# YukinoriMatsuoka/indy-plenum

Hardware: AMD Instinct MI355X
Metric: Ed25519 verifies/sec at 1/8 MI355X (256B msgs) + % of INT32 VALU peak vs host CPU (higher is better)
Workload: dtype int32

## Files before the change

include/edv_measure.h:

```cpp
#ifndef EDV_MEASURE_H
#define EDV_MEASURE_H

#include <stdint.h>

#ifdef __cplusplus
extern "C" {
#endif

int edv_time_batch_dev(const uint8_t *d_sigs, const uint8_t *d_pks, const uint8_t *d_msgs,
                       const uint64_t *d_msg_off, uint64_t msg_base, uint64_t n, uint8_t *d_accept, int device,
                       int iters, float *ms_out);

int edv_profile_batch_dev(const uint8_t *d_sigs, const uint8_t *d_pks, const uint8_t *d_msgs,
                          const uint64_t *d_msg_off, uint64_t msg_base, uint64_t n, uint8_t *d_accept, int device,
                          int iters, float *ms_prep, float *ms_main);

int edv_profile_batch_dev_flush(const uint8_t *d_sigs, const uint8_t *d_pks, const uint8_t *d_msgs,
                                const uint64_t *d_msg_off, uint64_t msg_base, uint64_t n, uint8_t *d_accept,
                                int device, int iters, uint64_t flush_bytes, float *ms_prep, float *ms_flush,
                                float *ms_main);

int edv_profile_prep_sides(const uint8_t *d_sigs, const uint8_t *d_pks, const uint8_t *d_msgs,
                           const uint64_t *d_msg_off, uint64_t msg_base, uint64_t n, uint8_t *d_accept, int device,
                           int iters, float ms[5]);

int edv_test_fail_async(int device, int64_t ticket);

#define EDV_PROBE_FE_MUL 1
#define EDV_PROBE_FE_SQ 2
#define EDV_PROBE_FE_SQ2 3
#define EDV_PROBE_FE_SQ_FLOOR 4
#define EDV_PROBE_FE_TOBYTES 5
#define EDV_PROBE_FE_FROMBYTES 6
#define EDV_PROBE_FE_INVERT_SAFEGCD 7
#define EDV_PROBE_FE_POW22523 8
#define EDV_PROBE_SC_REDUCE 9
#define EDV_PROBE_HALF_SCALARS 10
#define EDV_PROBE_RECODE5 11
#define EDV_PROBE_APPROX_DIV 12
#define EDV_PROBE_FDIV_FLOOR 13
#define EDV_PROBE_EUCLID_DIV 14
#define EDV_PROBE_GE_FROMBYTES 15
#define EDV_PROBE_QUAD_SQ_SHIFT 16
#define EDV_PROBE_QUAD_DBL 17
#define EDV_PROBE_QUAD_ADD 18
#define EDV_PROBE_QUAD_CACHED 19
#define EDV_PROBE_QUAD_CACHED_SIGNED 20
#define EDV_PROBE_SC_MULADD 21
#define EDV_PROBE_RECODE8 22
#define EDV_PROBE_SCALARMULT_BASE 23
#define EDV_PROBE_GE_P3_TOBYTES 24
int edv_probe_math(int device, int op, const void *in, uint64_t in_stride, void *out, uint64_t out_stride, uint64_t n);

#define EDV_STAGE_CAP 4096
#define EDV_STAGE_SENTINEL 0xA5
#define EDV_STAGE_BUCKETS 1u
#define EDV_STAGE_SPLIT 2u
#define EDV_STAGE_PRIO 4u
#define EDV_TABLE_SET_COMPACT 0
#define EDV_TABLE_SET_LARGE 1
#define EDV_TABLE_SET_COMB 2
int edv_probe_prep_state(int device, const uint8_t *sigs, const uint8_t *pks, const uint8_t *msgs,
                         const uint64_t *msg_off, uint64_t n, int set, int side0, int nsides, uint32_t flags,
                         uint32_t *dig, uint8_t *alive, int32_t *atab, int32_t *rtab, uint32_t *perm,
                         uint8_t *accept, uint64_t *cap);
int edv_probe_main_state(int device, uint64_t n, uint64_t cap, const uint32_t *dig, const uint8_t *alive,
                         const int32_t *atab, const int32_t *rtab, const uint32_t *perm, uint32_t flags,
                         uint8_t *accept);
int edv_probe_table(int device, int set, const int32_t *tj, uint64_t n, int32_t *out);

#define EDV_LAT_RTL 0
#define EDV_LAT_QUAD 1
int edv_probe_latency_phase1(int device, int kernel, int set, const uint8_t *sigs, const uint8_t *pks,
                             const uint8_t *msgs, const uint64_t *msg_off, uint64_t n, uint32_t *dig, int32_t *pt,
                             uint8_t *ok, uint8_t *accept);
int edv_probe_latency_walk(int device, int kernel, uint64_t n, uint64_t slots, const uint32_t *dig, const int32_t *pt,
                           const uint8_t *ok, uint32_t flags, uint8_t *accept);

#ifdef __cplusplus
}
#endif
#endif
```

indy-plenum_amd/csrc/edv_hostcheck.cpp:

```cpp
#define EDV_CHAIN_FLOOR 1
#include <stdint.h>
#include <string.h>
#include <vector>
#include "edv_verify_core.h"
#include "edv_sha256.h"
#include "edv_merkle.h"
#include "edv_ledger.h"
#include "edv_tables.h"
#include "edv_hostplan.h"
#include "edv_selftest_cases.h"
#include "edv_probe_ops.h"

using namespace edv;

namespace {
struct HostATab {
  ge_cached t[kAEntries];
  int staged = 0;
  void store(int e, const ge_cached& c) { t[e] = c; }
  ge_cached load(int e) const { return t[e]; }
  void stage(int e) { staged = e; }
  ge_cached fetch() const { return t[staged]; }
};
struct HostBTab {
// ... 139 lines not shown
  bool neg = false;
  half_scalars(h, a, u, neg);
  store_words(a32, a, 8);
  store_words(u32, u, 8);
  return neg ? 1 : 0;
}
int hc_probe_math(int op, const void* in, uint64_t in_stride, void* out, uint64_t out_stride, uint64_t n) {
  const ProbeSize sz = probe_size(op);
  if (!sz.in || probe_is_quad(op) || in_stride < sz.in || out_stride < sz.out || (in_stride & 3) || (out_stride & 3))
    return -1;
  for (uint64_t i = 0; i < n; i++) {
    const uint32_t* x = reinterpret_cast<const uint32_t*>(static_cast<const uint8_t*>(in) + i * in_stride);
    uint32_t* y = reinterpret_cast<uint32_t*>(static_cast<uint8_t*>(out) + i * out_stride);
    switch (op) {
#define HC_PROBE_CASE(OP) case OP: probe_lane_op<OP>(x, y); break;
      HC_PROBE_CASE(EDV_PROBE_FE_MUL)
      HC_PROBE_CASE(EDV_PROBE_FE_SQ)
      HC_PROBE_CASE(EDV_PROBE_FE_SQ2)
      HC_PROBE_CASE(EDV_PROBE_FE_SQ_FLOOR)
      HC_PROBE_CASE(EDV_PROBE_FE_TOBYTES)
      HC_PROBE_CASE(EDV_PROBE_FE_FROMBYTES)
      HC_PROBE_CASE(EDV_PROBE_FE_INVERT_SAFEGCD)
      HC_PROBE_CASE(EDV_PROBE_FE_POW22523)
      HC_PROBE_CASE(EDV_PROBE_SC_REDUCE)
      HC_PROBE_CASE(EDV_PROBE_HALF_SCALARS)
      HC_PROBE_CASE(EDV_PROBE_RECODE5)
      HC_PROBE_CASE(EDV_PROBE_APPROX_DIV)
      HC_PROBE_CASE(EDV_PROBE_FDIV_FLOOR)
      HC_PROBE_CASE(EDV_PROBE_EUCLID_DIV)
      HC_PROBE_CASE(EDV_PROBE_GE_FROMBYTES)
      HC_PROBE_CASE(EDV_PROBE_SC_MULADD)
      HC_PROBE_CASE(EDV_PROBE_RECODE8)
      HC_PROBE_CASE(EDV_PROBE_GE_P3_TOBYTES)
#undef HC_PROBE_CASE
      case EDV_PROBE_SCALARMULT_BASE: probe_scalarmult_base(x, y, comb()); break;
      default: return -1;
    }
  }
  return 0;
}
static_assert(kAEntries * 40 == 360, "a slot's table is 9 entries of 4 x 10 limbs");
int hc_stage_prep(const uint8_t* sigs, const uint8_t* pks, const uint8_t* msgs, const uint64_t* off, uint64_t n,
                  int bits, int side0, int nsides, int buckets, uint64_t cap, uint32_t* dig, uint8_t* alive,
                  int32_t* atab, int32_t* rtab, uint32_t* perm, uint8_t* accept) {
  if ((bits != kBBits && bits != kBBitsCompact) || n > cap || side0 < 0 || nsides < 1 || side0 + nsides > 3) return -1;
  const HostBTab& bt = btab(bits);
  if (buckets) {
    auto bucket = [&](uint64_t i) {
      const uint64_t nb = (64 + (off[i + 1] - off[i]) + 17 + 127) / 128;
      return nb < 63 ? nb : uint64_t(63);
    };
    uint64_t k = 0;
    bool one = true;
    for (uint64_t i = 1; i < n; i++) one = one && bucket(i) == bucket(0);
    for (uint64_t b = 0; b < 64 && !one; b++)
      for (uint64_t i = 0; i < n; i++)
        if (bucket(i) == b) perm[k++] = uint32_t(i);
    for (uint64_t i = 0; one && i < n; i++) perm[i] = uint32_t(i);
  }
  for (uint64_t j = 0; j < n; j++) {
    const uint64_t i = buckets ? perm[j] : j;
    uint32_t R[8], S[8], A[8];
    load_words(R, sigs + 64 * i, 8);
    load_words(S, sigs + 64 * i + 32, 8);
    load_words(A, pks + 32 * i, 8);
    for (int side = side0; side < side0 + nsides; side++) {
// ... 492 lines not shown
```

indy-plenum_amd/csrc/edv_math.h:

```cpp
#pragma once
#include <stdint.h>

#if defined(__HIPCC__)
#include <hip/hip_runtime.h>
#define EDV_HD __host__ __device__ __forceinline__
#else
#define EDV_HD inline
#endif

namespace edv {

struct fe { int32_t v[10]; };

EDV_HD fe fe_d() { return fe{{56195235, 13857412, 51736253, 6949390, 114729, 24766616, 60832955, 30306712, 48412415, 21499315}}; }
EDV_HD fe fe_d2() { return fe{{45281625, 27714825, 36363642, 13898781, 229458, 15978800, 54557047, 27058993, 29715967, 9444199}}; }
EDV_HD fe fe_sqrtm1() { return fe{{34513072, 25610706, 9377949, 3500415, 12389472, 33281959, 41962654, 31548777, 326685, 11406482}}; }

EDV_HD fe fe_zero() { return fe{{0, 0, 0, 0, 0, 0, 0, 0, 0, 0}}; }
EDV_HD fe fe_one() { return fe{{1, 0, 0, 0, 0, 0, 0, 0, 0, 0}}; }

EDV_HD fe fe_add(const fe& f, const fe& g) {
  fe h;
#pragma unroll
  for (int i = 0; i < 10; i++) h.v[i] = f.v[i] + g.v[i];
// ... 17 lines not shown
  for (int i = 0; i < 10; i++) h.v[i] = take_b ? b.v[i] : a.v[i];
  return h;
}

template <int W>
EDV_HD int32_t carry_step(int64_t h, int64_t& next) {
  const int64_t t = h + (int64_t(1) << (W - 1));
  next += t >> W;
  return int32_t(uint32_t(t) & ((1u << W) - 1)) - (1 << (W - 1));
}

EDV_HD fe fe_carry64(int64_t h0, int64_t h1, int64_t h2, int64_t h3, int64_t h4, int64_t h5, int64_t h6,
                     int64_t h7, int64_t h8, int64_t h9) {
  h0 = carry_step<26>(h0, h1);
  h4 = carry_step<26>(h4, h5);
  h1 = carry_step<25>(h1, h2);
  h5 = carry_step<25>(h5, h6);
  h2 = carry_step<26>(h2, h3);
  h6 = carry_step<26>(h6, h7);
  h3 = carry_step<25>(h3, h4);
  h7 = carry_step<25>(h7, h8);
  h4 = carry_step<26>(h4, h5);
  h8 = carry_step<26>(h8, h9);
  int64_t c9 = 0;
  h9 = carry_step<25>(h9, c9);
  h0 += c9 * 19;
  h0 = carry_step<26>(h0, h1);
  return fe{{int32_t(h0), int32_t(h1), int32_t(h2), int32_t(h3), int32_t(h4), int32_t(h5), int32_t(h6),
             int32_t(h7), int32_t(h8), int32_t(h9)}};
}

EDV_HD constexpr int64_t col_bias(int k) { return (k & 1) ? (int64_t(1) << 24) : (int64_t(1) << 25); }
#if defined(__HIP_DEVICE_COMPILE__)
__constant__ int64_t c_col_bias[3] = {int64_t(1) << 25, int64_t(1) << 24, 0};
EDV_HD int64_t bias_reg(int k) { return c_col_bias[k & 1]; }
EDV_HD int64_t zero_reg() { return c_col_bias[2]; }
#else
EDV_HD int64_t bias_reg(int k) { return col_bias(k); }
EDV_HD int64_t zero_reg() { return 0; }
#endif
template <int W>
EDV_HD int32_t carry_biased(int64_t t, int64_t& next) {
  next += t >> W;
  return int32_t(uint32_t(t) & ((1u << W) - 1)) - (1 << (W - 1));
}
EDV_HD fe fe_carry64_biased(int64_t h0, int64_t h1, int64_t h2, int64_t h3, int64_t h4, int64_t h5, int64_t h6,
                            int64_t h7, int64_t h8, int64_t h9) {
  h0 = carry_biased<26>(h0, h1);
  h1 = carry_biased<25>(h1, h2);
  h2 = carry_biased<26>(h2, h3);
  h3 = carry_biased<25>(h3, h4);
  h4 = carry_biased<26>(h4, h5);
  h5 = carry_biased<25>(h5, h6);
  h6 = carry_biased<26>(h6, h7);
  h7 = carry_biased<25>(h7, h8);
  h8 = carry_biased<26>(h8, h9);
  int64_t c9 = 0;
  h9 = carry_biased<25>(h9, c9);
  h0 += c9 * 19;
  h0 = carry_step<26>(h0, h1);
  return fe{{int32_t(h0), int32_t(h1), int32_t(h2), int32_t(h3), int32_t(h4), int32_t(h5), int32_t(h6),
             int32_t(h7), int32_t(h8), int32_t(h9)}};
}

EDV_HD void sched_fence() {
#if defined(__HIP_DEVICE_COMPILE__) && !defined(EDV_NO_SCHED_FENCE)
  __builtin_amdgcn_sched_barrier(0);
#endif
}

struct fe_mul_cols {
  int32_t f[10], g[10], g19[10], f2[10], f38_9;
  EDV_HD fe_mul_cols(const fe& ff, const fe& gg) {
#pragma unroll
    for (int i = 0; i < 10; i++) {
      f[i] = ff.v[i];
      g[i] = gg.v[i];
      g19[i] = 19 * gg.v[i];
      f2[i] = (i & 1) ? 2 * ff.v[i] : ff.v[i];
    }
    f38_9 = 38 * ff.v[9];
  }
  EDV_HD int64_t col(int k, int64_t start) const {
    int64_t acc = 0;
#pragma unroll
    for (int i = 0; i < 10; i++) {
      const int j = k - i;
      const bool f9w = (i == 9) && (j < 0) && ((j + 10) & 1);
      const int32_t a = f9w ? f38_9 : ((k & 1) == 0) ? f2[i] : f[i];
      const int32_t b = f9w ? g[j + 10] : (j >= 0) ? g[j] : g19[j + 10];
      acc = int64_t(a) * int64_t(b) + ((i == 0) ? start : acc);
    }
    return acc;
  }
};
EDV_HD fe fe_mul(const fe& f, const fe& g) {
  sched_fence();
  const fe_mul_cols cols(f, g);
  int64_t h[10];
#pragma unroll
  for (int k = 0; k < 10; k++) h[k] = cols.col(k, bias_reg(k));
  const fe r = fe_carry64_biased(h[0], h[1], h[2], h[3], h[4], h[5], h[6], h[7], h[8], h[9]);
  sched_fence();
  return r;
}

struct sq_split { int8_t x, y; };
constexpr sq_split kSqSplit[2][10][10] = {
    {
        {{1, 1}, {1, 2}, {1, 2}, {2, 1}, {2, 1}, {2, 1}, {2, 1}, {2, 1}, {2, 1}, {2, 1}},
        {{0, 0}, {1, 2}, {2, 1}, {2, 2}, {2, 1}, {2, 2}, {1, 2}, {2, 2}, {2, 1}, {2, 38}},
        {{0, 0}, {0, 0}, {1, 1}, {1, 2}, {2, 1}, {1, 2}, {1, 2}, {1, 2}, {2, 19}, {1, 38}},
        {{0, 0}, {0, 0}, {0, 0}, {1, 2}, {2, 1}, {2, 2}, {2, 1}, {2, 38}, {2, 19}, {2, 38}},
        {{0, 0}, {0, 0}, {0, 0}, {0, 0}, {1, 1}, {1, 2}, {2, 19}, {1, 38}, {2, 19}, {1, 38}},
        {{0, 0}, {0, 0}, {0, 0}, {0, 0}, {0, 0}, {19, 2}, {2, 19}, {2, 38}, {2, 19}, {2, 38}},
        {{0, 0}, {0, 0}, {0, 0}, {0, 0}, {0, 0}, {0, 0}, {19, 1}, {1, 38}, {2, 19}, {1, 38}},
        {{0, 0}, {0, 0}, {0, 0}, {0, 0}, {0, 0}, {0, 0}, {0, 0}, {1, 38}, {2, 19}, {2, 38}},
        {{0, 0}, {0, 0}, {0, 0}, {0, 0}, {0, 0}, {0, 0}, {0, 0}, {0, 0}, {1, 19}, {1, 38}},
        {{0, 0}, {0, 0}, {0, 0}, {0, 0}, {0, 0}, {0, 0}, {0, 0}, {0, 0}, {0, 0}, {1, 38}},
    },
    {
        {{1, 2}, {1, 4}, {2, 2}, {1, 4}, {2, 2}, {2, 2}, {2, 2}, {2, 2}, {2, 2}, {1, 4}},
        {{0, 0}, {4, 1}, {4, 1}, {8, 1}, {4, 1}, {8, 1}, {1, 4}, {4, 2}, {4, 1}, {8, 19}},
        {{0, 0}, {0, 0}, {2, 1}, {1, 4}, {2, 2}, {4, 1}, {2, 2}, {4, 1}, {4, 19}, {4, 19}},
        {{0, 0}, {0, 0}, {0, 0}, {1, 4}, {1, 4}, {4, 2}, {1, 4}, {4, 38}, {4, 19}, {4, 38}},
// ... 78 lines not shown
    c = t >> w;
  }
  c9 = c;
#else
  int64_t h[10];
  fe_sq_cols<false, false>(f, h);
  o[0] = carry_floor<26>(h[0], h[1]);
  o[1] = carry_floor<25>(h[1], h[2]);
  o[2] = carry_floor<26>(h[2], h[3]);
  o[3] = carry_floor<25>(h[3], h[4]);
  o[4] = carry_floor<26>(h[4], h[5]);
  o[5] = carry_floor<25>(h[5], h[6]);
  o[6] = carry_floor<26>(h[6], h[7]);
  o[7] = carry_floor<25>(h[7], h[8]);
  o[8] = carry_floor<26>(h[8], h[9]);
  o[9] = carry_floor<25>(h[9], c9);
#endif
  int64_t t0 = int64_t(o[0]) + 19 * c9, t1 = o[1];
  o[0] = carry_floor<26>(t0, t1);
  o[1] = int32_t(t1);
  const fe r{{o[0], o[1], o[2], o[3], o[4], o[5], o[6], o[7], o[8], o[9]}};
  sched_fence();
  return r;
}
EDV_HD fe fe_sq2(const fe& f) {
  sched_fence();
  int64_t h[10];
  fe_sq_cols<true>(f, h);
  const fe r = fe_carry64_biased(h[0], h[1], h[2], h[3], h[4], h[5], h[6], h[7], h[8], h[9]);
  sched_fence();
  return r;
}

EDV_HD fe fe_carry32(const fe& f) {
  int64_t h[10];
#pragma unroll
  for (int i = 0; i < 10; i++) h[i] = f.v[i];
  return fe_carry64(h[0], h[1], h[2], h[3], h[4], h[5], h[6], h[7], h[8], h[9]);
}

EDV_HD void fe_tobytes(uint32_t w[8], const fe& f) {
  int32_t h[10];
#pragma unroll
  for (int i = 0; i < 10; i++) h[i] = f.v[i];
  int32_t q = (19 * h[9] + (1 << 24)) >> 25;
#pragma unroll
  for (int i = 0; i < 10; i++) q = (h[i] + q) >> ((i & 1) ? 25 : 26);
  h[0] += 19 * q;
#pragma unroll
  for (int i = 0; i < 9; i++) {
    const int s = (i & 1) ? 25 : 26;
    const int32_t c = h[i] >> s;
    h[i + 1] += c;
    h[i] -= c * (1 << s);
  }
  h[9] &= (1 << 25) - 1;
  const uint32_t u0 = h[0], u1 = h[1], u2 = h[2], u3 = h[3], u4 = h[4], u5 = h[5], u6 = h[6], u7 = h[7],
                 u8 = h[8], u9 = h[9];
  w[0] = u0 | (u1 << 26);
  w[1] = (u1 >> 6) | (u2 << 19);
  w[2] = (u2 >> 13) | (u3 << 13);
  w[3] = (u3 >> 19) | (u4 << 6);
  w[4] = u5 | (u6 << 25);
  w[5] = (u6 >> 7) | (u7 << 19);
  w[6] = (u7 >> 13) | (u8 << 12);
  w[7] = (u8 >> 20) | (u9 << 6);
// ... 158 lines not shown
#pragma unroll 1
  for (int it = 0; it < 20; it++) {
    int32_t t[4];
    eta = divsteps_30(eta, uint32_t(f.v[0]), uint32_t(g.v[0]), t);
    update_de(d, e, t);
    update_fg(f, g, t);
  }
  const int64_t sgn = (f.v[8] >> 31) | 1;
  constexpr int kPos[10] = {0, 26, 51, 77, 102, 128, 153, 179, 204, 230};
  int64_t h[10] = {0, 0, 0, 0, 0, 0, 0, 0, 0, 0};
#pragma unroll
  for (int i = 0; i < 9; i++) {
    const int pos = 30 * i;
    int k = 0;
#pragma unroll
    for (int j = 0; j < 10; j++)
      if (kPos[j] <= pos) k = j;
    h[k] += (sgn * int64_t(d.v[i])) * (int64_t(1) << (pos - kPos[k]));
  }
  return fe_carry64(h[0], h[1], h[2], h[3], h[4], h[5], h[6], h[7], h[8], h[9]);
}

struct ge_p2 { fe X, Y, Z; };
struct ge_p3 { fe X, Y, Z, T; };
struct ge_p1p1 { fe X, Y, Z, T; };
struct ge_cached { fe YpX, YmX, Z, T2d; };
struct ge_precomp { fe ypx, ymx, xy2d; };

EDV_HD ge_p2 ge_p2_identity() { return ge_p2{fe_zero(), fe_one(), fe_one()}; }
EDV_HD ge_p3 ge_p3_identity() { return ge_p3{fe_zero(), fe_one(), fe_one(), fe_zero()}; }
EDV_HD ge_cached ge_cached_identity() { return ge_cached{fe_one(), fe_one(), fe_one(), fe_zero()}; }
EDV_HD ge_precomp ge_precomp_identity() { return ge_precomp{fe_one(), fe_one(), fe_zero()}; }

EDV_HD ge_p2 ge_p1p1_to_p2(const ge_p1p1& p) {
  return ge_p2{fe_mul(p.X, p.T), fe_mul(p.Z, p.Y), fe_mul(p.Z, p.T)};
}
EDV_HD ge_p3 ge_p1p1_to_p3(const ge_p1p1& p) {
  return ge_p3{fe_mul(p.X, p.T), fe_mul(p.Z, p.Y), fe_mul(p.Z, p.T), fe_mul(p.X, p.Y)};
}
EDV_HD ge_p2 ge_p3_to_p2(const ge_p3& p) { return ge_p2{p.X, p.Y, p.Z}; }
EDV_HD ge_cached ge_p3_to_cached(const ge_p3& p) {
  return ge_cached{fe_add(p.Y, p.X), fe_sub(p.Y, p.X), p.Z, fe_mul(p.T, fe_d2())};
}

EDV_HD ge_p1p1 ge_p2_dbl(const ge_p2& p) {
  ge_p1p1 r;
  const fe XX = fe_sq(p.X);
  const fe YY = fe_sq(p.Y);
  const fe B = fe_sq2(p.Z);
  const fe A = fe_sq(fe_add(p.X, p.Y));
  r.Y = fe_add(YY, XX);
  r.Z = fe_sub(YY, XX);
  r.X = fe_sub(A, r.Y);
  r.T = fe_sub(B, r.Z);
  return r;
}
EDV_HD ge_p1p1 ge_add(const ge_p3& p, const ge_cached& q) {
  ge_p1p1 r;
  const fe A = fe_mul(fe_add(p.Y, p.X), q.YpX);
  const fe B = fe_mul(fe_sub(p.Y, p.X), q.YmX);
  const fe C = fe_mul(q.T2d, p.T);
  const fe ZZ = fe_mul(p.Z, q.Z);
  const fe D = fe_add(ZZ, ZZ);
  r.X = fe_sub(A, B);
  r.Y = fe_add(A, B);
  r.Z = fe_add(D, C);
  r.T = fe_sub(D, C);
  return r;
}
EDV_HD ge_p1p1 ge_madd(const ge_p3& p, const ge_precomp& q) {
  ge_p1p1 r;
  const fe A = fe_mul(fe_add(p.Y, p.X), q.ypx);
  const fe B = fe_mul(fe_sub(p.Y, p.X), q.ymx);
  const fe C = fe_mul(q.xy2d, p.T);
  const fe D = fe_add(p.Z, p.Z);
  r.X = fe_sub(A, B);
  r.Y = fe_add(A, B);
  r.Z = fe_add(D, C);
  r.T = fe_sub(D, C);
  return r;
}
EDV_HD void fe_cswap_mask(fe& a, fe& b, int32_t m) {
#pragma unroll
  for (int i = 0; i < 10; i++) {
    const int32_t t = (a.v[i] ^ b.v[i]) & m;
    a.v[i] ^= t;
    b.v[i] ^= t;
  }
}
EDV_HD fe fe_cneg_mask(const fe& a, int32_t m) {
  fe h;
#pragma unroll
  for (int i = 0; i < 10; i++) h.v[i] = (a.v[i] ^ m) - m;
  return h;
}
// ... 267 lines not shown
```

indy-plenum_amd/csrc/edv_probe.hip:

```cpp
#define EDV_CHAIN_FLOOR 1
#include <hip/hip_runtime.h>
#include <stdint.h>

#include "edv_probe.h"

namespace edv {
namespace {

template <int OP>
__global__ __launch_bounds__(256) void edv_probe_lane_kernel(const uint8_t* in, uint64_t in_stride, uint8_t* out,
                                                             uint64_t out_stride, uint64_t n) {
  const uint64_t i = uint64_t(blockIdx.x) * 256 + threadIdx.x;
  if (i >= n) return;
  probe_lane_op<OP>(reinterpret_cast<const uint32_t*>(in + i * in_stride),
                    reinterpret_cast<uint32_t*>(out + i * out_stride));
}

__global__ __launch_bounds__(256) void edv_probe_comb_kernel(const uint8_t* in, uint64_t in_stride, uint8_t* out,
                                                             uint64_t out_stride, uint64_t n, const int32_t* comb) {
  const uint64_t i = uint64_t(blockIdx.x) * 256 + threadIdx.x;
  if (i >= n) return;
  probe_scalarmult_base(reinterpret_cast<const uint32_t*>(in + i * in_stride),
                        reinterpret_cast<uint32_t*>(out + i * out_stride), GlobalComb{comb});
}

}

hipError_t launch_probe_lane(hipStream_t s, int op, const uint8_t* in, uint64_t in_stride, uint8_t* out,
                             uint64_t out_stride, uint64_t n, const int32_t* comb) {
  const dim3 grid(unsigned((n + 255) / 256)), block(256);
  switch (op) {
    case EDV_PROBE_SCALARMULT_BASE:
      if (!comb) return hipErrorInvalidValue;
      edv_probe_comb_kernel<<<grid, block, 0, s>>>(in, in_stride, out, out_stride, n, comb);
      break;
#define EDV_PROBE_CASE(OP) \
  case OP: edv_probe_lane_kernel<OP><<<grid, block, 0, s>>>(in, in_stride, out, out_stride, n); break;
    EDV_PROBE_CASE(EDV_PROBE_FE_MUL)
    EDV_PROBE_CASE(EDV_PROBE_FE_SQ)
    EDV_PROBE_CASE(EDV_PROBE_FE_SQ2)
    EDV_PROBE_CASE(EDV_PROBE_FE_SQ_FLOOR)
    EDV_PROBE_CASE(EDV_PROBE_FE_TOBYTES)
    EDV_PROBE_CASE(EDV_PROBE_FE_FROMBYTES)
    EDV_PROBE_CASE(EDV_PROBE_FE_INVERT_SAFEGCD)
    EDV_PROBE_CASE(EDV_PROBE_FE_POW22523)
    EDV_PROBE_CASE(EDV_PROBE_SC_REDUCE)
    EDV_PROBE_CASE(EDV_PROBE_HALF_SCALARS)
    EDV_PROBE_CASE(EDV_PROBE_RECODE5)
    EDV_PROBE_CASE(EDV_PROBE_APPROX_DIV)
    EDV_PROBE_CASE(EDV_PROBE_FDIV_FLOOR)
    EDV_PROBE_CASE(EDV_PROBE_EUCLID_DIV)
    EDV_PROBE_CASE(EDV_PROBE_GE_FROMBYTES)
    EDV_PROBE_CASE(EDV_PROBE_SC_MULADD)
    EDV_PROBE_CASE(EDV_PROBE_RECODE8)
    EDV_PROBE_CASE(EDV_PROBE_GE_P3_TOBYTES)
#undef EDV_PROBE_CASE
    default: return hipErrorInvalidValue;
  }
  return hipGetLastError();
}

}
```

indy-plenum_amd/csrc/edv_probe_ops.h:

```cpp
#pragma once
#include "edv_verify_core.h"
#include "../../include/edv_measure.h"

namespace edv {

struct ProbeSize {
  uint32_t in, out;
};
EDV_HD constexpr ProbeSize probe_size(int op) {
  switch (op) {
    case EDV_PROBE_FE_MUL: return ProbeSize{80, 40};
    case EDV_PROBE_FE_SQ:
    case EDV_PROBE_FE_SQ2:
    case EDV_PROBE_FE_SQ_FLOOR:
    case EDV_PROBE_FE_INVERT_SAFEGCD:
    case EDV_PROBE_FE_POW22523: return ProbeSize{40, 40};
    case EDV_PROBE_FE_TOBYTES: return ProbeSize{40, 32};
    case EDV_PROBE_FE_FROMBYTES: return ProbeSize{32, 40};
    case EDV_PROBE_SC_REDUCE: return ProbeSize{64, 32};
    case EDV_PROBE_HALF_SCALARS: return ProbeSize{32, 68};
    case EDV_PROBE_RECODE5: return ProbeSize{32, 36};
    case EDV_PROBE_APPROX_DIV:
    case EDV_PROBE_FDIV_FLOOR: return ProbeSize{16, 8};
    case EDV_PROBE_EUCLID_DIV: return ProbeSize{128, 64};
    case EDV_PROBE_GE_FROMBYTES: return ProbeSize{32, 172};
    case EDV_PROBE_QUAD_SQ_SHIFT: return ProbeSize{176, 160};
    case EDV_PROBE_QUAD_DBL:
    case EDV_PROBE_QUAD_CACHED: return ProbeSize{160, 160};
    case EDV_PROBE_QUAD_ADD: return ProbeSize{320, 160};
    case EDV_PROBE_QUAD_CACHED_SIGNED: return ProbeSize{164, 160};
    case EDV_PROBE_SC_MULADD: return ProbeSize{96, 32};
    case EDV_PROBE_RECODE8: return ProbeSize{32, 32};
    case EDV_PROBE_SCALARMULT_BASE: return ProbeSize{32, 192};
    case EDV_PROBE_GE_P3_TOBYTES: return ProbeSize{160, 32};
    default: return ProbeSize{0, 0};
  }
}
EDV_HD constexpr bool probe_is_quad(int op) { return op >= EDV_PROBE_QUAD_SQ_SHIFT && op <= EDV_PROBE_QUAD_CACHED_SIGNED; }

EDV_HD fe probe_fe(const uint32_t* x) {
  fe f;
#pragma unroll
  for (int i = 0; i < 10; i++) f.v[i] = int32_t(x[i]);
  return f;
}
EDV_HD void probe_put(uint32_t* y, const fe& f) {
#pragma unroll
  for (int i = 0; i < 10; i++) y[i] = uint32_t(f.v[i]);
}
EDV_HD ge_p3 probe_p3(const uint32_t* x) { return ge_p3{probe_fe(x), probe_fe(x + 10), probe_fe(x + 20), probe_fe(x + 30)}; }
EDV_HD void probe_put_p3(uint32_t* y, const ge_p3& p) {
  probe_put(y, p.X);
  probe_put(y + 10, p.Y);
  probe_put(y + 20, p.Z);
  probe_put(y + 30, p.T);
}
EDV_HD double probe_f64(const uint32_t* x) { return __builtin_bit_cast(double, pack64(x[0], x[1])); }
EDV_HD void probe_put_f64(uint32_t* y, double d) {
  const uint64_t b = __builtin_bit_cast(uint64_t, d);
  y[0] = uint32_t(b);
  y[1] = uint32_t(b >> 32);
}

template <int OP>
EDV_HD void probe_lane_op(const uint32_t* x, uint32_t* y) {
  if constexpr (OP == EDV_PROBE_FE_MUL) {
    probe_put(y, fe_mul(probe_fe(x), probe_fe(x + 10)));
  } else if constexpr (OP == EDV_PROBE_FE_SQ) {
    probe_put(y, fe_sq(probe_fe(x)));
  } else if constexpr (OP == EDV_PROBE_FE_SQ2) {
    probe_put(y, fe_sq2(probe_fe(x)));
  } else if constexpr (OP == EDV_PROBE_FE_SQ_FLOOR) {
    probe_put(y, fe_sq_floor(probe_fe(x)));
  } else if constexpr (OP == EDV_PROBE_FE_TOBYTES) {
    uint32_t w[8];
    fe_tobytes(w, probe_fe(x));
#pragma unroll
    for (int i = 0; i < 8; i++) y[i] = w[i];
  } else if constexpr (OP == EDV_PROBE_FE_FROMBYTES) {
    uint32_t w[8];
#pragma unroll
    for (int i = 0; i < 8; i++) w[i] = x[i];
    probe_put(y, fe_frombytes(w));
  } else if constexpr (OP == EDV_PROBE_FE_INVERT_SAFEGCD) {
    probe_put(y, fe_invert_safegcd(probe_fe(x)));
  } else if constexpr (OP == EDV_PROBE_FE_POW22523) {
    probe_put(y, fe_pow22523(probe_fe(x)));
  } else if constexpr (OP == EDV_PROBE_SC_REDUCE) {
    uint32_t w[16], o[8];
#pragma unroll
    for (int i = 0; i < 16; i++) w[i] = x[i];
    sc_reduce(o, w);
#pragma unroll
    for (int i = 0; i < 8; i++) y[i] = o[i];
  } else if constexpr (OP == EDV_PROBE_HALF_SCALARS) {
    uint32_t h[8], a[8], u[8];
#pragma unroll
    for (int i = 0; i < 8; i++) h[i] = x[i];
    bool neg = false;
    half_scalars(h, a, u, neg);
#pragma unroll
    for (int i = 0; i < 8; i++) { y[i] = a[i]; y[8 + i] = u[i]; }
    y[16] = neg ? 1u : 0u;
  } else if constexpr (OP == EDV_PROBE_RECODE5) {
    uint32_t s[8], d[8];
#pragma unroll
// ... 62 lines not shown
```

indy-plenum_amd/csrc/edv_verify.hip:

```cpp
#include <hip/hip_runtime.h>
#include <stdint.h>

#include "edv_verify_core.h"
#include "edv_kernels.h"
#include "edv_launch.h"
#include "edv_sha256.h"

using namespace edv;

namespace {

constexpr int kEntryPieces = 10;
constexpr int kLdsAWords = kEntryPieces * 256;
constexpr int kLdsWaveWords = 2 * kLdsAWords;
__device__ __forceinline__ void wait_staged() { asm volatile("s_waitcnt vmcnt(0)" ::: "memory"); }
struct LdsATab {
  const int32_t* slot;
  int32_t* lds;
  int lane;
  __device__ __forceinline__ void stage(int e) {
    const int32_t* g = slot + e * kEntryWords;
#pragma unroll
    for (int q = 0; q < kEntryPieces; q++)
      __builtin_amdgcn_global_load_lds(const_cast<int32_t*>(g + 4 * q), lds + q * 256, 16, 0, 0);
  }
  __device__ __forceinline__ ge_cached fetch() {
    wait_staged();
    int32_t t[4 * kEntryPieces];
#pragma unroll
    for (int q = 0; q < kEntryPieces; q++) {
      const int4 v = reinterpret_cast<const int4*>(lds + q * 256)[lane];
      t[4 * q] = v.x; t[4 * q + 1] = v.y; t[4 * q + 2] = v.z; t[4 * q + 3] = v.w;
// ... 2 lines not shown
#pragma unroll
    for (int l = 0; l < 10; l++) {
      c.YpX.v[l] = t[l]; c.YmX.v[l] = t[10 + l]; c.Z.v[l] = t[20 + l]; c.T2d.v[l] = t[30 + l];
    }
    return c;
  }
};
#define EDV_MAIN_BODY \
  const uint64_t j = uint64_t(blockIdx.x) * kBlock + threadIdx.x; \
  const bool live = j < a.n && a.st.alive[j] && a.st.alive[a.st.cap + j] && a.st.alive[2 * a.st.cap + j]; \
  const uint32_t* d = a.st.dig + j; \
  const uint64_t cap = a.st.cap; \
  const uint32_t wf = live ? d[uint64_t(kDigNwin) * cap] : 0; \
  int nwin = int(wf & 0xff); \
_Pragma("unroll") \
  for (int o = 32; o > 0; o >>= 1) nwin = max(nwin, __shfl_xor(nwin, o)); \
  nwin = __builtin_amdgcn_readfirstlane(nwin); \
  if (!live) return; \
  const uint64_t i = a.base + (a.st.perm ? a.st.perm[j] : j); \
  uint32_t da[8], db[8]; \
_Pragma("unroll") \
  for (int k = 0; k < 8; k++) { \
    da[k] = d[uint64_t(k) * cap]; \
    db[k] = d[uint64_t(8 + k) * cap]; \
  } \
_Pragma("unroll") \
  for (int k = 0; k < 8; k++) { \
    da[k] = uint32_t(opaque_i32(int32_t(da[k]))); \
    db[k] = uint32_t(opaque_i32(int32_t(db[k]))); \
  } \
  int32_t* wl = lds_main + (threadIdx.x >> 6) * kLdsWaveWords; \
  const int lane = int(threadIdx.x & 63); \
  LdsATab at{a.st.atab + j * kAWords, wl, lane}, rt{a.st.rtab + j * kAWords, wl + kLdsAWords, lane}; \
  a.accept[i] = main_one(da, db, nwin, (wf >> 8) & 1, at, rt) ? 1 : 0;

__global__ __launch_bounds__(kBlock) void edv_main_kernel(VerifyArgs a) {
  __shared__ int32_t lds_main[(kBlock / 64) * kLdsWaveWords];
  EDV_MAIN_BODY
}

constexpr int kSplitMainPrio = 2;
__global__ __launch_bounds__(kBlock) void edv_main_kernel_prio(VerifyArgs a) {
  __shared__ int32_t lds_main[(kBlock / 64) * kLdsWaveWords];
  __builtin_amdgcn_s_setprio(kSplitMainPrio);
  EDV_MAIN_BODY
}

__global__ __launch_bounds__(kBlock) void edv_sign_kernel(const uint32_t* seeds, const uint8_t* msgs,
                                                          const uint64_t* off, uint64_t msg_base, uint64_t n,
                                                          uint32_t* pks, uint32_t* sigs, const int32_t* comb) {
  const uint64_t i = uint64_t(blockIdx.x) * kBlock + threadIdx.x;
  if (i >= n) return;
  uint32_t seed[8], pk[8], sig[16];
  load_words(seed, seeds + 8 * i, 2);
  const uint64_t o0 = off[i] - msg_base, o1 = off[i + 1] - msg_base;
  sign_one(pk, sig, seed, msgs + o0, o1 - o0, GlobalComb{comb});
  uint4* po = reinterpret_cast<uint4*>(pks + 8 * i);
  uint4* so = reinterpret_cast<uint4*>(sigs + 16 * i);
  po[0] = make_uint4(pk[0], pk[1], pk[2], pk[3]);
  po[1] = make_uint4(pk[4], pk[5], pk[6], pk[7]);
#pragma unroll
  for (int k = 0; k < 4; k++) so[k] = make_uint4(sig[4 * k], sig[4 * k + 1], sig[4 * k + 2], sig[4 * k + 3]);
}

__global__ void edv_comb_kernel(int32_t* out) {
  const int t = threadIdx.x + blockIdx.x * blockDim.x;
  if (t < kCombRows * kCombEntries) comb_entry(out + t * kBStride, t / kCombEntries, t % kCombEntries);
// ... 127 lines not shown
```

indy-plenum_amd/csrc/edv_verify_core.h:

```cpp
#pragma once
#include "edv_math.h"

namespace edv {

constexpr int kAWin = 4;
constexpr int kAWindows = (255 + kAWin - 1) / kAWin;
constexpr int kAEntries = (1 << (kAWin - 1)) + 1;
constexpr int kBBits = 22;
constexpr int kBTables = (253 + kBBits - 1) / kBBits;
constexpr int kBEntries = (1 << (kBBits - 1)) + 1;
constexpr int kBBitsCompact = 16;
constexpr int kBTablesCompact = (253 + kBBitsCompact - 1) / kBBitsCompact;
constexpr int kBEntriesCompact = (1 << (kBBitsCompact - 1)) + 1;
static_assert(253 - kBBits * (kBTables - 1) <= kBBits - 1, "top [S]B digit out of table range");
static_assert(253 - kBBitsCompact * (kBTablesCompact - 1) <= kBBitsCompact - 1, "top [S]B digit out of table range");
struct SbShape {
  int bits, tables, entries;
};
EDV_HD constexpr SbShape sb_large() { return SbShape{kBBits, kBTables, kBEntries}; }
EDV_HD constexpr SbShape sb_compact() { return SbShape{kBBitsCompact, kBTablesCompact, kBEntriesCompact}; }
constexpr int kCombEntries = 129;
constexpr int kBStride = 32;

EDV_HD int mx(int a, int b) { return a > b ? a : b; }
// ... 523 lines not shown
  auto next_digit = [&](bool top) {
    int e = int(s[0] & ((1u << bits) - 1)) + carry;
    shr256_var(s, bits);
    carry = top ? 0 : (e + (1 << (bits - 1))) >> bits;
    return e - carry * (1 << bits);
  };
  int dt = next_digit(sh.tables == 1);
  bt.stage(0, dt < 0 ? -dt : dt);
#pragma unroll 1
  for (int t = 0; t < sh.tables; t++) {
    const ge_precomp e = ge_precomp_cneg(bt.fetch(), dt < 0);
    if (t + 1 < sh.tables) {
      dt = next_digit(t + 2 == sh.tables);
      bt.stage(t + 1, dt < 0 ? -dt : dt);
    }
    q = ge_p1p1_to_p3(ge_madd(q, e));
  }
}
template <class BTab>
EDV_HD bool rpoint_q(const uint32_t R[8], const uint32_t S[8], BTab& bt, ge_p3& q) {
  if (!ge_is_canonical(R) || has_small_order(R)) return false;
  if (!ge_frombytes_negate(q, R)) return false;
  add_sb(q, S, bt);
  return true;
}
template <class ATab, class BTab>
EDV_HD bool prep_rpoint(const uint32_t R[8], const uint32_t S[8], ATab& tab, BTab& bt) {
  ge_p3 q;
  if (!rpoint_q(R, S, bt, q)) return false;
  build_table_projective(tab, q, bt);
  return true;
}

template <class ATab>
EDV_HD bool main_one(uint32_t da[8], uint32_t db[8], int nwin, bool negR, ATab& at, ATab& rt) {
  constexpr int kTop = kAWin * (kAWindows - 1);
  constexpr int kTopShl = 32 - kAWin - (kTop - 224);
#pragma unroll 1
  for (int k = nwin; k < kAWindows; k++) {
    shl256<kAWin>(da);
    shl256<kAWin>(db);
  }
  ge_p2 acc = ge_p2_identity();
#pragma unroll 1
  for (int w = nwin - 1; w >= 0; --w) {
    const int dA = int32_t(da[7] << kTopShl) >> (32 - kAWin);
    const int dR = int32_t(db[7] << kTopShl) >> (32 - kAWin);
    shl256<kAWin>(da);
    shl256<kAWin>(db);
    at.stage(dA < 0 ? -dA : dA);
    rt.stage(dR < 0 ? -dR : dR);
    ge_p3 p3;
    if (w == nwin - 1) {
      p3 = ge_p3_identity();
    } else {
#pragma unroll 1
      for (int d = 0; d < kAWin - 1; d++) acc = ge_p1p1_to_p2(ge_p2_dbl(acc));
      p3 = ge_p1p1_to_p3(ge_p2_dbl(acc));
    }
    const ge_cached ea = at.fetch();
    p3 = ge_p1p1_to_p3(ge_add(p3, ge_cached_cneg(ea, dA < 0)));
    const ge_cached er = rt.fetch();
    acc = ge_p1p1_to_p2(ge_add(p3, ge_cached_cneg(er, (dR < 0) != negR)));
  }
  return fe_iszero(acc.X) && fe_iszero(fe_carry32(fe_sub(acc.Y, acc.Z)));
}

template <class ATab, class BTab>
EDV_HD bool verify_one(const uint32_t R[8], const uint32_t S[8], const uint32_t A[8], const uint8_t* m, uint64_t mlen,
                       ATab& at, ATab& rt, BTab& bt) {
  PrepDigits pd;
  if (!prep_one(R, S, A, m, mlen, pd)) return false;
  if (!prep_point(A, at) || !prep_rpoint(R, S, rt, bt)) return false;
  return main_one(pd.da, pd.db, pd.nwin, pd.negR, at, rt);
}

constexpr int kCombRows = 32;
EDV_HD void comb_entry(int32_t* o, int i, int j) {
  const uint32_t Bw[8] = {0x66666658u, 0x66666666u, 0x66666666u, 0x66666666u,
                          0x66666666u, 0x66666666u, 0x66666666u, 0x66666666u};
  ge_p3 nB;
  ge_frombytes_negate(nB, Bw);
  ge_p3 base{fe_neg(nB.X), nB.Y, nB.Z, fe_neg(nB.T)};
  for (int k = 0; k < 8 * i; k++) base = ge_p1p1_to_p3(ge_p2_dbl(ge_p3_to_p2(base)));
  const ge_cached bc = ge_p3_to_cached(base);
  ge_p3 acc = ge_p3_identity();
  for (int bit = 7; bit >= 0; bit--) {
    acc = ge_p1p1_to_p3(ge_p2_dbl(ge_p3_to_p2(acc)));
    if ((j >> bit) & 1) acc = ge_p1p1_to_p3(ge_add(acc, bc));
  }
  const fe zi = fe_invert(acc.Z);
  const fe x = fe_mul(acc.X, zi), y = fe_mul(acc.Y, zi);
  const fe ypx = fe_carry32(fe_add(y, x)), ymx = fe_carry32(fe_sub(y, x));
  const fe xy2d = fe_mul(fe_mul(x, y), fe_d2());
  for (int l = 0; l < 10; l++) { o[l] = ypx.v[l]; o[10 + l] = ymx.v[l]; o[20 + l] = xy2d.v[l]; }
  o[30] = 0;
// ... 65 lines not shown
```

indy-plenum_amd/edv.py:

```python
import ctypes
import os
import threading

import numpy as np

from . import _edvhost

_HERE = os.path.dirname(os.path.abspath(__file__))
LIB_PATH = os.environ.get("EDV_LIB", os.path.join(_HERE, "libedv.so"))
MEASURE_LIB_PATH = os.path.join(_HERE, "libedv_measure.so")
MEASUREMENT_TAG = "MEASUREMENT-ONLY"

EDV_OK = 0
EDV_E_ARG = -1
EDV_E_NODEV = -2
EDV_E_HIP = -3
EDV_E_OOM = -4
EDV_E_BUSY = -5
EDV_E_SELFTEST = -6
TABLES_AUTO, TABLES_COMPACT, TABLES_LARGE = 0, 1, 2
SELFTEST_RTL, SELFTEST_TWO_WALK, SELFTEST_BATCH = 1, 2, 4
SELFTEST_ALL = 7
PREPARE_ASYNC = 1
FLAG_UNIFORM_LENGTH = 1
# ... 730 lines not shown
def profile_device(d_sigs, d_pks, d_msgs, d_off, n, d_accept, device=0, iters=1, msg_base=0):
    a, b = ctypes.c_float(0), ctypes.c_float(0)
    _mcheck(measure_lib().edv_profile_batch_dev(d_sigs, d_pks, d_msgs, d_off, msg_base, n, d_accept, device, iters,
                                                ctypes.byref(a), ctypes.byref(b)))
    return float(a.value), float(b.value)


def profile_device_flush(d_sigs, d_pks, d_msgs, d_off, n, d_accept, device=0, iters=1, flush_bytes=0, msg_base=0):
    a, f, b = ctypes.c_float(0), ctypes.c_float(0), ctypes.c_float(0)
    _mcheck(measure_lib().edv_profile_batch_dev_flush(d_sigs, d_pks, d_msgs, d_off, msg_base, n, d_accept, device,
                                                      iters, flush_bytes, ctypes.byref(a), ctypes.byref(f),
                                                      ctypes.byref(b)))
    return float(a.value), float(f.value), float(b.value)


PREP_SIDE_KEYS = ("hash_side", "a_side", "r_side", "all_three", "point_sides")


def profile_prep_sides(d_sigs, d_pks, d_msgs, d_off, n, d_accept, device=0, iters=1, msg_base=0) -> dict:
    ms = (ctypes.c_float * 5)()
    _mcheck(measure_lib().edv_profile_prep_sides(d_sigs, d_pks, d_msgs, d_off, msg_base, n, d_accept, device, iters,
                                                 ms))
    return dict(zip(PREP_SIDE_KEYS, (float(x) for x in ms)))


PROBE_OPS = {
    "fe_mul": (1, 80, 40), "fe_sq": (2, 40, 40), "fe_sq2": (3, 40, 40), "fe_sq_floor": (4, 40, 40),
    "fe_tobytes": (5, 40, 32), "fe_frombytes": (6, 32, 40), "fe_invert_safegcd": (7, 40, 40),
    "fe_pow22523": (8, 40, 40), "sc_reduce": (9, 64, 32), "half_scalars": (10, 32, 68), "recode5": (11, 32, 36),
    "approx_div": (12, 16, 8), "fdiv_floor": (13, 16, 8), "euclid_div": (14, 128, 64),
    "ge_frombytes": (15, 32, 172), "quad_sq_shift": (16, 176, 160), "quad_dbl": (17, 160, 160),
    "quad_add": (18, 320, 160), "quad_cached": (19, 160, 160), "quad_cached_signed": (20, 164, 160),
    "sc_muladd": (21, 96, 32), "recode8": (22, 32, 32), "scalarmult_base": (23, 32, 192),
    "ge_p3_tobytes": (24, 160, 32),
}


def probe_math(op, cases, device=0):
    code, nin, nout = PROBE_OPS[op]
    cases = np.ascontiguousarray(cases, dtype=np.uint8)
    if cases.ndim != 2 or cases.shape[1] != nin:
        raise ValueError("probe {}: cases must be (n, {}) bytes".format(op, nin))
    out = np.zeros((cases.shape[0], nout), np.uint8)
    _mcheck(measure_lib().edv_probe_math(device, code, cases.ctypes.data, nin, out.ctypes.data, nout,
                                         cases.shape[0]))
    return out


STAGE_CAP = 4096
STAGE_SENTINEL = 0xA5
STAGE_BUCKETS, STAGE_SPLIT, STAGE_PRIO = 1, 2, 4
TABLE_SETS = {"compact": 0, "large": 1, "comb": 2}
A_WORDS = 360
DIG_WORDS = 17


def probe_prep_state(sigs, pks, msgs, offsets, table_set="compact", buckets=False, split=False, side0=0, nsides=3,
                     device=0) -> dict:
    sigs, pks, msgs = (np.ascontiguousarray(np.frombuffer(bytes(x), np.uint8) if isinstance(x, (bytes, bytearray))
                                            else x, dtype=np.uint8) for x in (sigs, pks, msgs))
    off = np.ascontiguousarray(offsets, dtype=np.uint64)
    n = len(off) - 1
    if sigs.size != 64 * n or pks.size != 32 * n or (n and msgs.size < int(off[-1])):
        raise ValueError("prep probe: sigs n x 64, pks n x 32, msgs at least offsets[n] bytes")
    cap = ctypes.c_uint64(0)
    st = {"dig": np.full((DIG_WORDS, STAGE_CAP), STAGE_SENTINEL * 0x01010101, np.uint32),
          "alive": np.full((3, STAGE_CAP), STAGE_SENTINEL, np.uint8),
# ... 88 lines not shown
```

Measured before the change: 99.41 million.

## Interleave pairs of field multiplies and squarings in the double-scalar walk

Adds paired field multiply and square routines that accumulate two independent products column by column with a shared biased carry chain. They replace the separate fe_mul/fe_sq calls in point doubling, addition and coordinate conversions in the main verify walk, enabled by default via EDV_PAIR_PRODUCTS. The aim is more instruction-level parallelism and fewer carry passes per product, at the cost of more live registers, which can lower occupancy or cause spills.

```diff
diff --git a/include/edv_measure.h b/include/edv_measure.h
--- a/include/edv_measure.h
+++ b/include/edv_measure.h
@@ -50,6 +50,9 @@
 #define EDV_PROBE_RECODE8 22
 #define EDV_PROBE_SCALARMULT_BASE 23
 #define EDV_PROBE_GE_P3_TOBYTES 24
+#define EDV_PROBE_FE_MUL_PAIR 32
+#define EDV_PROBE_FE_SQ_PAIR 33
+#define EDV_PROBE_FE_SQ2_SQ_PAIR 34
 int edv_probe_math(int device, int op, const void *in, uint64_t in_stride, void *out, uint64_t out_stride, uint64_t n);
 
 #define EDV_STAGE_CAP 4096
diff --git a/indy-plenum_amd/csrc/edv_hostcheck.cpp b/indy-plenum_amd/csrc/edv_hostcheck.cpp
--- a/indy-plenum_amd/csrc/edv_hostcheck.cpp
+++ b/indy-plenum_amd/csrc/edv_hostcheck.cpp
@@ -195,6 +195,9 @@
       HC_PROBE_CASE(EDV_PROBE_SC_MULADD)
       HC_PROBE_CASE(EDV_PROBE_RECODE8)
       HC_PROBE_CASE(EDV_PROBE_GE_P3_TOBYTES)
+      HC_PROBE_CASE(EDV_PROBE_FE_MUL_PAIR)
+      HC_PROBE_CASE(EDV_PROBE_FE_SQ_PAIR)
+      HC_PROBE_CASE(EDV_PROBE_FE_SQ2_SQ_PAIR)
 #undef HC_PROBE_CASE
       case EDV_PROBE_SCALARMULT_BASE: probe_scalarmult_base(x, y, comb()); break;
       default: return -1;
diff --git a/indy-plenum_amd/csrc/edv_math.h b/indy-plenum_amd/csrc/edv_math.h
--- a/indy-plenum_amd/csrc/edv_math.h
+++ b/indy-plenum_amd/csrc/edv_math.h
@@ -73,12 +73,14 @@
 
 EDV_HD constexpr int64_t col_bias(int k) { return (k & 1) ? (int64_t(1) << 24) : (int64_t(1) << 25); }
 #if defined(__HIP_DEVICE_COMPILE__)
-__constant__ int64_t c_col_bias[3] = {int64_t(1) << 25, int64_t(1) << 24, 0};
+__constant__ int64_t c_col_bias[4] = {int64_t(1) << 25, int64_t(1) << 24, 0, (int64_t(1) << 25) + (int64_t(1) << 50)};
 EDV_HD int64_t bias_reg(int k) { return c_col_bias[k & 1]; }
 EDV_HD int64_t zero_reg() { return c_col_bias[2]; }
+EDV_HD int64_t pair_bias_reg() { return c_col_bias[3]; }
 #else
 EDV_HD int64_t bias_reg(int k) { return col_bias(k); }
 EDV_HD int64_t zero_reg() { return 0; }
+EDV_HD int64_t pair_bias_reg() { return col_bias(0) + (col_bias(1) << 26); }
 #endif
 template <int W>
 EDV_HD int32_t carry_biased(int64_t t, int64_t& next) {
@@ -122,16 +124,18 @@
     }
     f38_9 = 38 * ff.v[9];
   }
+  static constexpr int count(int) { return 10; }
+  EDV_HD int64_t term(int k, int i) const {
+    const int j = k - i;
+    const bool f9w = (i == 9) && (j < 0) && ((j + 10) & 1);
+    const int32_t a = f9w ? f38_9 : ((k & 1) == 0) ? f2[i] : f[i];
+    const int32_t b = f9w ? g[j + 10] : (j >= 0) ? g[j] : g19[j + 10];
+    return int64_t(a) * int64_t(b);
+  }
   EDV_HD int64_t col(int k, int64_t start) const {
     int64_t acc = 0;
 #pragma unroll
-    for (int i = 0; i < 10; i++) {
-      const int j = k - i;
-      const bool f9w = (i == 9) && (j < 0) && ((j + 10) & 1);
-      const int32_t a = f9w ? f38_9 : ((k & 1) == 0) ? f2[i] : f[i];
-      const int32_t b = f9w ? g[j + 10] : (j >= 0) ? g[j] : g19[j + 10];
-      acc = int64_t(a) * int64_t(b) + ((i == 0) ? start : acc);
-    }
+    for (int i = 0; i < 10; i++) acc = term(k, i) + ((i == 0) ? start : acc);
     return acc;
   }
 };
@@ -276,6 +280,81 @@
   return r;
 }
 
+template <bool DOUBLE>
+struct fe_sq_terms {
+  const fe& f;
+  static constexpr int count(int k) { return (k & 1) ? 5 : 6; }
+  EDV_HD int64_t term(int k, int t) const {
+    int64_t p = 0;
+    int n = 0;
+#pragma unroll
+    for (int i = 0; i < 10; i++) {
+#pragma unroll
+      for (int j = i; j < 10; j++) {
+        if ((i + j) % 10 != k) continue;
+        if (n++ != t) continue;
+        const sq_split m = kSqSplit[DOUBLE ? 1 : 0][i][j];
+        p = int64_t(f.v[i] * int32_t(m.x)) * int64_t(f.v[j] * int32_t(m.y));
+      }
+    }
+    return p;
+  }
+};
+EDV_HD int64_t pair_add(int64_t x, int64_t p) {
+#if defined(__HIP_DEVICE_COMPILE__)
+  return __builtin_annotation(x + p, "edv_pin");
+#else
+  return x + p;
+#endif
+}
+EDV_HD constexpr int imax(int a, int b) { return a > b ? a : b; }
+template <class T0, class T1>
+EDV_HD void fe_pair_sum(const T0& p0, const T1& p1, fe& r0, fe& r1) {
+  int64_t c0 = 0, c1 = 0;
+#pragma unroll
+  for (int k = 0; k < 10; k++) {
+    const bool odd = k & 1;
+    const int w = odd ? 25 : 26;
+    int64_t a0 = odd ? c0 : pair_bias_reg(), a1 = odd ? c1 : pair_bias_reg();
+#pragma unroll
+    for (int t = 0; t < imax(T0::count(k), T1::count(k)); t++) {
+      if (t < T0::count(k)) a0 = pair_add(a0, p0.term(k, t));
+      if (t < T1::count(k)) a1 = pair_add(a1, p1.term(k, t));
+    }
+    if (!odd && k > 0) {
+      a0 += c0;
+      a1 += c1;
+    }
+    r0.v[k] = int32_t(uint32_t(a0) & ((1u << w) - 1)) - (1 << (w - 1));
+    r1.v[k] = int32_t(uint32_t(a1) & ((1u << w) - 1)) - (1 << (w - 1));
+    c0 = a0 >> w;
+    c1 = a1 >> w;
+  }
+  int64_t h0 = r0.v[0] + 19 * c0, h1 = r0.v[1];
+  r0.v[0] = carry_step<26>(h0, h1);
+  r0.v[1] = int32_t(h1);
+  h0 = r1.v[0] + 19 * c1, h1 = r1.v[1];
+  r1.v[0] = carry_step<26>(h0, h1);
+  r1.v[1] = int32_t(h1);
+}
+struct fe_pair { fe a, b; };
+EDV_HD fe_pair fe_mul_pair(const fe& f0, const fe& g0, const fe& f1, const fe& g1) {
+  sched_fence();
+  const fe_mul_cols m0(f0, g0), m1(f1, g1);
+  fe_pair r;
+  fe_pair_sum(m0, m1, r.a, r.b);
+  sched_fence();
+  return r;
+}
+template <bool D0 = false, bool D1 = false>
+EDV_HD fe_pair fe_sq_pair(const fe& f0, const fe& f1) {
+  sched_fence();
+  fe_pair r;
+  fe_pair_sum(fe_sq_terms<D0>{f0}, fe_sq_terms<D1>{f1}, r.a, r.b);
+  sched_fence();
+  return r;
+}
+
 EDV_HD fe fe_carry32(const fe& f) {
   int64_t h[10];
 #pragma unroll
@@ -500,35 +579,62 @@
 EDV_HD ge_cached ge_cached_identity() { return ge_cached{fe_one(), fe_one(), fe_one(), fe_zero()}; }
 EDV_HD ge_precomp ge_precomp_identity() { return ge_precomp{fe_one(), fe_one(), fe_zero()}; }
 
+template <bool PAIR = false>
 EDV_HD ge_p2 ge_p1p1_to_p2(const ge_p1p1& p) {
-  return ge_p2{fe_mul(p.X, p.T), fe_mul(p.Z, p.Y), fe_mul(p.Z, p.T)};
-}
+  if constexpr (PAIR) {
+    const fe_pair xz = fe_mul_pair(p.X, p.T, p.Z, p.T);
+    return ge_p2{xz.a, fe_mul(p.Z, p.Y), xz.b};
+  } else {
+    return ge_p2{fe_mul(p.X, p.T), fe_mul(p.Z, p.Y), fe_mul(p.Z, p.T)};
+  }
+}
+template <bool PAIR = false>
 EDV_HD ge_p3 ge_p1p1_to_p3(const ge_p1p1& p) {
-  return ge_p3{fe_mul(p.X, p.T), fe_mul(p.Z, p.Y), fe_mul(p.Z, p.T), fe_mul(p.X, p.Y)};
+  if constexpr (PAIR) {
+    const fe_pair xz = fe_mul_pair(p.X, p.T, p.Z, p.T), yt = fe_mul_pair(p.Z, p.Y, p.X, p.Y);
+    return ge_p3{xz.a, yt.a, xz.b, yt.b};
+  } else {
+    return ge_p3{fe_mul(p.X, p.T), fe_mul(p.Z, p.Y), fe_mul(p.Z, p.T), fe_mul(p.X, p.Y)};
+  }
 }
 EDV_HD ge_p2 ge_p3_to_p2(const ge_p3& p) { return ge_p2{p.X, p.Y, p.Z}; }
 EDV_HD ge_cached ge_p3_to_cached(const ge_p3& p) {
   return ge_cached{fe_add(p.Y, p.X), fe_sub(p.Y, p.X), p.Z, fe_mul(p.T, fe_d2())};
 }
 
+template <bool PAIR = false>
 EDV_HD ge_p1p1 ge_p2_dbl(const ge_p2& p) {
   ge_p1p1 r;
-  const fe XX = fe_sq(p.X);
-  const fe YY = fe_sq(p.Y);
-  const fe B = fe_sq2(p.Z);
-  const fe A = fe_sq(fe_add(p.X, p.Y));
+  fe XX, YY, B, A;
+  if constexpr (PAIR) {
+    const fe_pair xy = fe_sq_pair(p.X, p.Y), ba = fe_sq_pair<true, false>(p.Z, fe_add(p.X, p.Y));
+    XX = xy.a; YY = xy.b; B = ba.a; A = ba.b;
+  } else {
+    XX = fe_sq(p.X);
+    YY = fe_sq(p.Y);
+    B = fe_sq2(p.Z);
+    A = fe_sq(fe_add(p.X, p.Y));
+  }
   r.Y = fe_add(YY, XX);
   r.Z = fe_sub(YY, XX);
   r.X = fe_sub(A, r.Y);
   r.T = fe_sub(B, r.Z);
   return r;
 }
+template <bool PAIR = false>
 EDV_HD ge_p1p1 ge_add(const ge_p3& p, const ge_cached& q) {
   ge_p1p1 r;
-  const fe A = fe_mul(fe_add(p.Y, p.X), q.YpX);
-  const fe B = fe_mul(fe_sub(p.Y, p.X), q.YmX);
-  const fe C = fe_mul(q.T2d, p.T);
-  const fe ZZ = fe_mul(p.Z, q.Z);
+  fe A, B, C, ZZ;
+  if constexpr (PAIR) {
+    const fe_pair ab = fe_mul_pair(fe_add(p.Y, p.X), q.YpX, fe_sub(p.Y, p.X), q.YmX);
+    const fe_pair cz = fe_mul_pair(q.T2d, p.T, p.Z, q.Z);
+    A = ab.a; B = ab.b; C = cz.a; ZZ = cz.b;
+  } else {
+    A = fe_mul(fe_add(p.Y, p.X), q.YpX);
+    B = fe_mul(fe_sub(p.Y, p.X), q.YmX);
+    C = fe_mul(q.T2d, p.T);
+    ZZ = fe_mul(p.Z, q.Z);
+  }
   const fe D = fe_add(ZZ, ZZ);
   r.X = fe_sub(A, B);
   r.Y = fe_add(A, B);
diff --git a/indy-plenum_amd/csrc/edv_probe.hip b/indy-plenum_amd/csrc/edv_probe.hip
--- a/indy-plenum_amd/csrc/edv_probe.hip
+++ b/indy-plenum_amd/csrc/edv_probe.hip
@@ -54,6 +54,9 @@
     EDV_PROBE_CASE(EDV_PROBE_SC_MULADD)
     EDV_PROBE_CASE(EDV_PROBE_RECODE8)
     EDV_PROBE_CASE(EDV_PROBE_GE_P3_TOBYTES)
+    EDV_PROBE_CASE(EDV_PROBE_FE_MUL_PAIR)
+    EDV_PROBE_CASE(EDV_PROBE_FE_SQ_PAIR)
+    EDV_PROBE_CASE(EDV_PROBE_FE_SQ2_SQ_PAIR)
 #undef EDV_PROBE_CASE
     default: return hipErrorInvalidValue;
   }
diff --git a/indy-plenum_amd/csrc/edv_probe_ops.h b/indy-plenum_amd/csrc/edv_probe_ops.h
--- a/indy-plenum_amd/csrc/edv_probe_ops.h
+++ b/indy-plenum_amd/csrc/edv_probe_ops.h
@@ -33,6 +33,9 @@
     case EDV_PROBE_RECODE8: return ProbeSize{32, 32};
     case EDV_PROBE_SCALARMULT_BASE: return ProbeSize{32, 192};
     case EDV_PROBE_GE_P3_TOBYTES: return ProbeSize{160, 32};
+    case EDV_PROBE_FE_MUL_PAIR: return ProbeSize{160, 80};
+    case EDV_PROBE_FE_SQ_PAIR:
+    case EDV_PROBE_FE_SQ2_SQ_PAIR: return ProbeSize{80, 80};
     default: return ProbeSize{0, 0};
   }
 }
@@ -72,6 +75,14 @@
     probe_put(y, fe_sq2(probe_fe(x)));
   } else if constexpr (OP == EDV_PROBE_FE_SQ_FLOOR) {
     probe_put(y, fe_sq_floor(probe_fe(x)));
+  } else if constexpr (OP == EDV_PROBE_FE_MUL_PAIR) {
+    const fe_pair r = fe_mul_pair(probe_fe(x), probe_fe(x + 10), probe_fe(x + 20), probe_fe(x + 30));
+    probe_put(y, r.a);
+    probe_put(y + 10, r.b);
+  } else if constexpr (OP == EDV_PROBE_FE_SQ_PAIR || OP == EDV_PROBE_FE_SQ2_SQ_PAIR) {
+    const fe_pair r = fe_sq_pair<OP == EDV_PROBE_FE_SQ2_SQ_PAIR, false>(probe_fe(x), probe_fe(x + 10));
+    probe_put(y, r.a);
+    probe_put(y + 10, r.b);
   } else if constexpr (OP == EDV_PROBE_FE_TOBYTES) {
     uint32_t w[8];
     fe_tobytes(w, probe_fe(x));
diff --git a/indy-plenum_amd/csrc/edv_verify.hip b/indy-plenum_amd/csrc/edv_verify.hip
--- a/indy-plenum_amd/csrc/edv_verify.hip
+++ b/indy-plenum_amd/csrc/edv_verify.hip
@@ -1,3 +1,6 @@
+#ifndef EDV_PAIR_PRODUCTS
+#define EDV_PAIR_PRODUCTS 1
+#endif
 #include <hip/hip_runtime.h>
 #include <stdint.h>
 
@@ -66,7 +69,7 @@
   int32_t* wl = lds_main + (threadIdx.x >> 6) * kLdsWaveWords; \
   const int lane = int(threadIdx.x & 63); \
   LdsATab at{a.st.atab + j * kAWords, wl, lane}, rt{a.st.rtab + j * kAWords, wl + kLdsAWords, lane}; \
-  a.accept[i] = main_one(da, db, nwin, (wf >> 8) & 1, at, rt) ? 1 : 0;
+  a.accept[i] = main_one<EDV_PAIR_PRODUCTS != 0>(da, db, nwin, (wf >> 8) & 1, at, rt) ? 1 : 0;
 
 __global__ __launch_bounds__(kBlock) void edv_main_kernel(VerifyArgs a) {
   __shared__ int32_t lds_main[(kBlock / 64) * kLdsWaveWords];
diff --git a/indy-plenum_amd/csrc/edv_verify_core.h b/indy-plenum_amd/csrc/edv_verify_core.h
--- a/indy-plenum_amd/csrc/edv_verify_core.h
+++ b/indy-plenum_amd/csrc/edv_verify_core.h
@@ -579,7 +579,7 @@
   return true;
 }
 
-template <class ATab>
+template <bool PAIR = false, class ATab>
 EDV_HD bool main_one(uint32_t da[8], uint32_t db[8], int nwin, bool negR, ATab& at, ATab& rt) {
   constexpr int kTop = kAWin * (kAWindows - 1);
   constexpr int kTopShl = 32 - kAWin - (kTop - 224);
@@ -602,13 +602,13 @@
       p3 = ge_p3_identity();
     } else {
 #pragma unroll 1
-      for (int d = 0; d < kAWin - 1; d++) acc = ge_p1p1_to_p2(ge_p2_dbl(acc));
-      p3 = ge_p1p1_to_p3(ge_p2_dbl(acc));
+      for (int d = 0; d < kAWin - 1; d++) acc = ge_p1p1_to_p2<PAIR>(ge_p2_dbl<PAIR>(acc));
+      p3 = ge_p1p1_to_p3<PAIR>(ge_p2_dbl<PAIR>(acc));
     }
     const ge_cached ea = at.fetch();
-    p3 = ge_p1p1_to_p3(ge_add(p3, ge_cached_cneg(ea, dA < 0)));
+    p3 = ge_p1p1_to_p3<PAIR>(ge_add<PAIR>(p3, ge_cached_cneg(ea, dA < 0)));
     const ge_cached er = rt.fetch();
-    acc = ge_p1p1_to_p2(ge_add(p3, ge_cached_cneg(er, (dR < 0) != negR)));
+    acc = ge_p1p1_to_p2<PAIR>(ge_add<PAIR>(p3, ge_cached_cneg(er, (dR < 0) != negR)));
   }
   return fe_iszero(acc.X) && fe_iszero(fe_carry32(fe_sub(acc.Y, acc.Z)));
 }
diff --git a/indy-plenum_amd/edv.py b/indy-plenum_amd/edv.py
--- a/indy-plenum_amd/edv.py
+++ b/indy-plenum_amd/edv.py
@@ -786,7 +786,8 @@
     "ge_frombytes": (15, 32, 172), "quad_sq_shift": (16, 176, 160), "quad_dbl": (17, 160, 160),
     "quad_add": (18, 320, 160), "quad_cached": (19, 160, 160), "quad_cached_signed": (20, 164, 160),
     "sc_muladd": (21, 96, 32), "recode8": (22, 32, 32), "scalarmult_base": (23, 32, 192),
-    "ge_p3_tobytes": (24, 160, 32),
+    "ge_p3_tobytes": (24, 160, 32), "fe_mul_pair": (32, 160, 80), "fe_sq_pair": (33, 80, 80),
+    "fe_sq2_sq_pair": (34, 80, 80),
 }
 
 
```

Result: no change. 99.87 million (median of 6 runs) (+0.5%).
